# DDMAL/text_alignment

Measured on AMD Instinct MI355X. Metric: nw_dp_cells_per_s, higher is better.
Workload: dtype int32; 1 GPU; affine-gap NW, 4096 problems of 4096x4096 per GPU per step, default scoring [8,-4,-7,-7,-3,0], two-phase (score fill + windowed traceback); parallelism=problems sharded x1, no data-path collective, distinct_problems=256

## Files before the change

include/text_alignment_amd.h:

```cpp
#ifndef TEXT_ALIGNMENT_AMD_H
#define TEXT_ALIGNMENT_AMD_H

#include <stdint.h>

#ifdef __cplusplus
extern "C" {
#endif

#define TA_OK 0
#define TA_EINVAL (-1)
#define TA_ERANGE (-2)
#define TA_EHIP (-3)
#define TA_ELIMIT (-4)

#define TA_NW_FILL 1u
#define TA_NW_TRACEBACK 2u
#define TA_NW_CODES8 4u
#define TA_NW_WIDE 8u
#define TA_NW_NARROW 16u
#define TA_NW_OPENS_SAME 32u
#define TA_NW_ALPHABET_SHIFT 8
#define TA_NW_ALPHABET(a) (((uint32_t)(a) & 0xFFu) << TA_NW_ALPHABET_SHIFT)
#define TA_NW_ROWS_SHIFT 20
#define TA_NW_ROWS(r) (((uint32_t)(r) & 0x7u) << TA_NW_ROWS_SHIFT)
// ... 44 lines not shown
                      uint8_t* ws, const int64_t* ws_off,
                      uint8_t* ops_out, const int64_t* ops_off, int32_t* ops_len,
                      int32_t max_n, int32_t max_m, int64_t score_bound,
                      uint32_t flags, int32_t band_w, const int32_t* band_u, int32_t* band_ok, void* stream);
int ta_nw2_batch_funnel(const int32_t* t_codes, const int64_t* t_off,
                        const int32_t* o_codes, const int64_t* o_off, int32_t nprob,
                        const int32_t* params, int32_t params_stride,
                        uint8_t* ws, const int64_t* ws_off,
                        uint8_t* ops_out, const int64_t* ops_off, int32_t* ops_len,
                        int32_t max_n, int32_t max_m, int64_t score_bound,
                        uint32_t flags, int32_t band_w, const int32_t* band_u, int32_t* band_ok,
                        const int32_t* band_x0, int32_t* band_cert, void* stream);
int ta_nw2_funnel_plan(const int32_t* n_arr, const int32_t* m_arr, int32_t nprob, const int32_t* params,
                       int32_t params_stride, int32_t w, int32_t big, int32_t* x0_out, int32_t* ranges_out,
                       int32_t ranges_cap, int32_t* out);
int32_t ta_nw2_funnel_suf(int32_t rn, int32_t rm, const int32_t* params, int32_t* ap_out);
int32_t ta_nw2_band_bound(int32_t n, int32_t m, const int32_t* params, int32_t w);
int ta_nw2_band_plan(const int32_t* n_arr, const int32_t* m_arr, int32_t nprob, const int32_t* params,
                     int32_t params_stride, uint32_t flags, int32_t band, int32_t* out, int32_t* u_out,
                     int32_t* ranges_out, int32_t ranges_cap);

int32_t ta_nw2_traceback_plan(int32_t nprob, int32_t params_stride, uint32_t flags);
int ta_nw2_phase1_plan(int32_t max_n, int32_t max_m, uint32_t flags, int32_t* out);
int ta_nw2_phase1_plan_batch(int32_t max_n, int32_t max_m, int32_t nprob, uint32_t flags, int32_t* out);

int64_t ta_nw_general_score_bytes(int32_t n);
int64_t ta_nw_general_ptr_bytes(int32_t n, int32_t m);
int ta_nw_general(const int32_t* t, int32_t n, const int32_t* o, int32_t m,
                  const double* params, const double* table, int32_t tm,
                  double* score_ws, uint8_t* ptr_ws,
// ... 313 lines not shown
```

text_alignment_amd/csrc/nw_band.h:

```cpp
#pragma once
#include <stdint.h>

#include "nw_cell.h"

namespace ta {

constexpr int kBandSentinel = -(1 << 24);
constexpr int kBandMaxLen = 32768;
static_assert(((int64_t)kBandSentinel - 2ll * kBandMaxLen * 128 - (1 << 21)) * 64 > INT32_MIN, "sentinel-derived values, encoded");
struct BandRange { int gl, gh; };
TA_HD BandRange band_groups(int n, int m, int w, int s) {
    const int ngroups = PtrLayout<4>::ngroups(m);
    const int lo = (m < n ? m - n : 0) - w, hi = (m > n ? m - n : 0) + w;
    const int i0 = s * 256 + 1;
    const int jmin = i0 + lo > 1 ? i0 + lo : 1;
    const int jmax = i0 + 255 + hi < m ? i0 + 255 + hi : m;
    const int kmin = jmin - 1, kmax = jmax - 1 + 63;
    int gl = kmin >= 2 ? ((kmin - 2) / 64) * 16 - 16 : 0;
    if (gl < 0) gl = 0;
    int gh = (kmax / 64) * 16 + 32;
    if (gh >= ngroups || gh <= gl) gh = ngroups;
    if (gl >= gh) gl = 0;
    return BandRange{gl, gh};
}
// ... 22 lines not shown
    f.a = prm[0] > prm[1] ? prm[0] : prm[1];
    f.cvi = prm[4] + (prm[2] > 0 ? prm[2] : 0);
    f.chi = prm[5] + (prm[3] > 0 ? prm[3] : 0);
    f.ap = f.a > f.cvi ? f.a : f.cvi;
    if (f.chi > f.ap) f.ap = f.chi;
    return f;
}
template <typename T>
TA_HD T funnel_suf(T rn, T rm, const FunnelSys& f) {
    const T d = rn < rm ? rn : rm;
    const T none = rn * (T)f.cvi + rm * (T)f.chi;
    const T most = d * (T)f.a + (rn - d) * (T)f.cvi + (rm - d) * (T)f.chi;
    return none > most ? none : most;
}

TA_HD BandRange funnel_raw(int n, int m, const FunnelSys& f, int w_outer, int s) {
    const int64_t den_h = 2ll * ((int64_t)f.a - f.cvi - f.chi), den_l = (int64_t)f.a - 2ll * f.cvi - 2ll * f.chi;
    if (f.a <= 0 || den_h <= 0 || den_l <= 0) return BandRange{-1, -1};
    const int ngroups = PtrLayout<4>::ngroups(m);
    const int w0 = (n < m ? n : m) / 32 > 128 ? (n < m ? n : m) / 32 : 128;
    const int64_t num = (int64_t)f.a * (n - 256 * s);
    const int64_t wh = (num + den_h - 1) / den_h + w0, wl = (num + den_l - 1) / den_l + w0;
    const int off_lo = m < n ? m - n : 0, off_hi = m > n ? m - n : 0;
    const int lo = wl < w_outer ? off_lo - (int)wl : off_lo - w_outer;
    const int hi = wh < w_outer ? off_hi + (int)wh : off_hi + w_outer;
    const int i0 = s * 256 + 1;
    const int jmin = i0 + lo > 1 ? i0 + lo : 1;
    const int jmax = i0 + 255 + hi < m ? i0 + 255 + hi : m;
    const int kmin = jmin - 1, kmax = jmax - 1 + 63;
    int gl = kmin >= 2 ? ((kmin - 2) / 64) * 16 - 16 : 0;
    if (gl < 0) gl = 0;
    int gh = (kmax / 64) * 16 + 32;
    if (gh >= ngroups || gh <= gl) gh = ngroups;
    if (gl >= gh) gl = 0;
    return BandRange{gl, gh};
}
TA_HD bool funnel_ok(int n, int m, const FunnelSys& f, int w_outer) {
    const int nstrips = PtrLayout<4>::nstrips(n), ngroups = PtrLayout<4>::ngroups(m);
    BandRange prev{0, 0};
    for (int s = 0; s < nstrips; ++s) {
        const BandRange r = funnel_raw(n, m, f, w_outer, s);
        if (r.gl < 0) return false;
        if (s > 0) {
            if (r.gl < prev.gl || r.gh < prev.gh) return false;
            if (r.gl > 0 && prev.gh < ngroups && 4 * r.gl + 2 > 4 * prev.gh - 63) return false;
        }
        prev = r;
    }
    return true;
}
TA_HD BandRange funnel_groups(int n, int m, const int32_t* prm, int w_outer, int s) {
    const FunnelSys f = funnel_sys(prm);
    return funnel_ok(n, m, f, w_outer) ? funnel_raw(n, m, f, w_outer, s) : band_groups(n, m, w_outer, s);
}
inline bool funnel_ranges(int n, int m, const int32_t* prm, int w_outer, BandRange* rg) {
    const FunnelSys f = funnel_sys(prm);
    const bool own = funnel_ok(n, m, f, w_outer);
    const int nstrips = PtrLayout<4>::nstrips(n);
    for (int s = 0; s < nstrips; ++s) rg[s] = own ? funnel_raw(n, m, f, w_outer, s) : band_groups(n, m, w_outer, s);
    return own;
}

TA_HD int funnel_jlo(const BandRange& r, int i) { return r.gl == 0 ? 1 : 4 * r.gl - ((i - 1) % 256) / 4 + 3; }
TA_HD int funnel_jhi(const BandRange& r, int i, int m) {
    if (r.gh == PtrLayout<4>::ngroups(m)) return m;
    const int j = 4 * r.gh - ((i - 1) % 256) / 4;
    return j < m ? j : m;
}
inline int64_t funnel_exit0(int n, int m, const int32_t* prm, const BandRange* rg) {
    const FunnelSys f = funnel_sys(prm);
    int64_t best = -(1ll << 40);
    auto out = [&](int i, int j) {
        if (i < 1 || i > n || j < 1 || j > m) return false;
        const BandRange& r = rg[(i - 1) / 256];
        return j < funnel_jlo(r, i) || j > funnel_jhi(r, i, m);
    };
    auto take = [&](int64_t db, int i, int j) {
        if (out(i, j)) best = bmax(best, db + f.ap + funnel_suf<int64_t>(n - i, m - j, f));
    };
    for (int j = 0; j <= m; ++j) { take(-j, 1, j); take(-j, 1, j + 1); }
    for (int i = 1; i <= n; ++i) { take(-i, i, 1); take(-i, i + 1, 1); }
    return best;
}

}
```

text_alignment_amd/csrc/nw_hw.h:

```cpp
#pragma once
#include <hip/hip_runtime.h>
#include <stdint.h>

#include "nw_cell.h"

namespace ta {

struct NwArgs {
    const int32_t* t_codes; const int64_t* t_off;
    const int32_t* o_codes; const int64_t* o_off;
    const int32_t* params; int32_t params_stride;
    uint8_t* ws; const int64_t* ws_off;
    uint8_t* ops_out; const int64_t* ops_off; int32_t* ops_len;
    int32_t nprob;
    int32_t wide_stride;
    int32_t apad;
    int32_t band_w;
    const int32_t* band_u;
    int32_t* band_ok;
    int32_t* band_cert;
};
constexpr int kCertWords = 4;

__device__ __forceinline__ int v_max3(int a, int b, int c) {
    int d;
    asm("v_max3_i32 %0, %1, %2, %3" : "=v"(d) : "v"(a), "v"(b), "v"(c));
    return d;
}
__device__ __forceinline__ int v_and_or_x(int a, int mask) {
    int d;
    asm("v_and_or_b32 %0, %1, %2, 21" : "=v"(d) : "v"(a), "s"(mask));
    return d;
}
__device__ __forceinline__ unsigned v_bfi3(unsigned a, unsigned b) {
    unsigned d;
// ... 176 lines not shown
```

text_alignment_amd/csrc/ta_nw2.hip:

```cpp
#include <hip/hip_runtime.h>
#include <stdint.h>
#include <array>
#include <atomic>
#include <map>
#include <type_traits>
#include <vector>

#include "nw_band.h"
#include "nw_cell.h"
#include "nw_hw.h"
#include "ta_common.h"

namespace ta {

#ifndef TA_CK_GROUPS
#define TA_CK_GROUPS 16
#endif
constexpr int kCkGroups = TA_CK_GROUPS;
static_assert(kCkGroups % 4 == 0 && kCkGroups >= 4, "whole blocks of four groups");
constexpr int kStateInts = 10;
constexpr int kWsRange = 0x7ffff000;

#ifndef TA_SUBROWS
#define TA_SUBROWS 2
// ... 55 lines not shown
};

__device__ __forceinline__ int wave_max_i32(int v) {
#pragma unroll
    for (int o = 32; o > 0; o >>= 1) v = max(v, __shfl_xor(v, o));
    return __builtin_amdgcn_readfirstlane(v);
}
template <int W, int MODE, bool SAMEGO, typename OC, int BAND = 0>
__global__ __launch_bounds__(W * 64, MODE == 1 ? 5 : 2) void nw_score_kernel(NwArgs a) {
    constexpr int R = 4;
    using L = PtrLayout<R>;
    constexpr int SPG = L::SPG;
    constexpr bool PROFILE = (MODE == 2);
    using LC = typename std::conditional<PROFILE, uint16_t, OC>::type;
    constexpr int CHK = 4;
    constexpr bool FUNNEL = BAND == 3;
    extern __shared__ __attribute__((aligned(16))) unsigned char smem[];

    int p = blockIdx.x;
    if constexpr (BAND == 2) {
        if (a.band_ok[p] != 0) return;
    }
    const int64_t t0 = a.t_off[p], o0 = a.o_off[p];
    const int n = (int)(a.t_off[p + 1] - t0);
    const int m = (int)(a.o_off[p + 1] - o0);
    if (n <= 0 || m <= 0) return;

    const int32_t* prm = a.params + (size_t)p * a.params_stride;
    const CellConsts c = make_consts(prm[0], prm[1], prm[2], prm[3], prm[4], prm[5]);
    RawRegs kr;
    kr.cmis = prm[1] - prm[4] - prm[5]; kr.cmat = prm[0] - prm[4] - prm[5];
// ... 38 lines not shown

    const uint64_t wsa = reinterpret_cast<uint64_t>(ws_p);
    unsigned char* const ws_u = reinterpret_cast<unsigned char*>(
        ((uint64_t)(uint32_t)__builtin_amdgcn_readfirstlane((int)(wsa >> 32)) << 32) |
        (uint32_t)__builtin_amdgcn_readfirstlane((int)(uint32_t)wsa));
    const __amdgpu_buffer_rsrc_t wsrc = __builtin_amdgcn_make_buffer_rsrc(ws_u, 0, kWsRange, 0x00020000);
    const int nstrips = ws.nstrips, ngroups = ws.ngroups;
    const int prev_wave = (wave + W - 1) % W;
    const int g_lo = (63 + SPG - 1) / SPG;
    const int g_hi = (steady_ok && ws.total < kWsRange) ? ngroups : 0;
    const bool from_zero = PROFILE && g_hi > 0 && prm[4] <= -1;
    int pass = 0;
    const FunnelSys fsys = funnel_sys(prm);
    bool fun_ok = false;
    if constexpr (FUNNEL) fun_ok = a.band_cert[kCertWords * p + 3] != 0;
    auto strip_range = [&](int s_) { return fun_ok ? funnel_raw(n, m, fsys, a.band_w, s_) : band_groups(n, m, a.band_w, s_); };
    auto exit_of = [&](int db_hat, int i, int j, int i2, int j2) {
        return db_hat + prm[4] * i + prm[5] * j + fsys.ap + funnel_suf<int>(n - i2, m - j2, fsys);
    };
    int ex_wave = -(1 << 30), cnt_wave = 0;

    for (int s = wave; s < nstrips; s += W, ++pass) {
        int D[R], V[R], H[R], tc[R];
        const int row0 = s * L::SR + lane * R;
#pragma unroll
        for (int r = 0; r < R; ++r) {
            const int i = row0 + r + 1;
            D[r] = raw_of(bnd_D_col0(c, i));
            H[r] = raw_of(bnd_H_col0(c, i)) + yadj;
            V[r] = from_zero ? -(1 << 28) : 0;
            tc[r] = (i <= n) ? a.t_codes[t0 + i - 1] : -1;
        }
        int dsave = raw_of(bnd_D_col0(c, row0));
// ... 130 lines not shown
                    if (sub_last) hvo[j] = make_int2(V[R - 1], D[R - 1]);
                }
            }
            publish(g);
        };

        int g = 0;
        if ((BAND == 1 || FUNNEL) && gl > 0) {
            g = gl;
            wait_span(gl);
            if constexpr (FUNNEL) {
                const int gl_above = strip_range(s - 1).gl;
                const int c_lo = gl_above == 0 ? 1 : gl_above * SPG - 60;
                const int c_hi = min(m, gl * SPG + 2), i0 = s * L::SR + 1;
                int ex = -(1 << 30);
                for (int j = c_lo + lane; j <= c_hi; j += 64) {
                    const int db = hvd[j].y;
                    ex = max(ex, exit_of(db, i0 - 1, j, i0, j));
                    if (j + 1 <= c_hi) ex = max(ex, exit_of(db, i0 - 1, j, i0, j + 1));
                }
                ex_wave = max(ex_wave, wave_max_i32(ex));
                if (lane == 31) hvo[gl * SPG - 31] = make_int2(kBandSentinel, kBandSentinel);
            }
        } else {
            wait_span(0);
            load_group(0);
            const int e1 = from_zero ? 0 : min(g_lo, ngroups);
            for (; g < e1; ++g) group_edge(g);
        }

        int g_end = g_hi & ~3;
        if constexpr (BAND == 1 || FUNNEL) {
            g_end = min(g_end, g_fin);
            if (cert_strip) g_end = min(g_end, ((m - 1 + cert_lane) / SPG) & ~3);
// ... 99 lines not shown
#pragma unroll
                for (int b = 0; b < kCkGroups / CHK; ++b) block();
            }
            while (g < g_end) {
                checkpoint(g);
                block();
            }
            if (g < g_fin) {
                if ((g % CHK) == 0) wait_span(g);
                load_group(g);
            } else {
                if constexpr (FUNNEL) {
                    if (g_fin < ngroups) {
                        const int jr = g_fin * SPG - lane;
                        int ex = -(1 << 30);
                        if (jr <= m) {
#pragma unroll
                            for (int r = 0; r < R; ++r) {
                                const int i = row0 + 1 + r;
                                if (i > n) continue;
                                if (jr + 1 <= m) ex = max(ex, exit_of(D[r], i, jr, i, jr + 1));
                                if (jr + 1 <= m && i + 1 <= n) ex = max(ex, exit_of(D[r], i, jr, i + 1, jr + 1));
                                if (r == R - 1 && lane < 63 && i + 1 <= n) ex = max(ex, exit_of(D[r], i, jr, i + 1, jr));
                            }
                        }
                        if (jr + 1 <= m && row0 + 1 <= n) ex = max(ex, exit_of(dsave, row0, jr, row0 + 1, jr + 1));
                        ex_wave = max(ex_wave, wave_max_i32(ex));
                        int2* const row31 = reinterpret_cast<int2*>(ws_p + ws.row(s * kSubRows + 1)) + 1;
                        if (lane < 3 && g_fin * SPG - 30 + lane <= m)
                            row31[g_fin * SPG - 30 + lane] = make_int2(kBandSentinel, kBandSentinel);
                        int2* const rowp = reinterpret_cast<int2*>(ws_p + ws.row(s * kSubRows + kSubRows)) + 1;
                        const int c_hi = min(m, strip_range(s + 1).gh * SPG + 4);
                        for (int col = g_fin * SPG - 62 + lane; col <= c_hi; col += 64)
                            rowp[col] = make_int2(kBandSentinel, kBandSentinel);
                    }
                }
                if constexpr (BAND == 1) {
                    if (g_fin < ngroups) {
                        int2* const rowp = reinterpret_cast<int2*>(ws_p + ws.row(s * kSubRows + kSubRows)) + 1;
                        const int c_hi = min(m, band_groups(n, m, a.band_w, s + 1).gh * SPG + 4);
                        for (int col = g_fin * SPG - 62 + lane; col <= c_hi; col += 64)
// ... 26 lines not shown
    const bool own = n > 0 && m > 0 && n <= kBandMaxLen && m <= kBandMaxLen &&
                     funnel_ok(n, m, funnel_sys(a.params + (size_t)p * a.params_stride), a.band_w);
    a.band_cert[kCertWords * p] = INT32_MIN;
    a.band_cert[kCertWords * p + 1] = x0[p];
    a.band_cert[kCertWords * p + 2] = 0;
    a.band_cert[kCertWords * p + 3] = own ? 1 : 0;
    a.band_ok[p] = 0;
}
__global__ __launch_bounds__(256) void nw_band_certify_kernel(NwArgs a) {
    const int p = blockIdx.x * 256 + threadIdx.x;
    if (p >= a.nprob) return;
    const int n = (int)(a.t_off[p + 1] - a.t_off[p]);
    const int32_t* c = a.band_cert + kCertWords * (size_t)p;
    const bool ok = n > 0 && c[2] == PtrLayout<4>::nstrips(n) && c[0] > a.band_u[p] && c[0] > c[1];
    a.band_ok[p] = ok ? 1 : 0;
}

constexpr int kChunk = kCkGroups;
constexpr int kChunkGroups = kChunk + 1;
constexpr int kChunkSteps = kChunkGroups * 4;
#ifndef TA_TB2_LANES
#define TA_TB2_LANES 32
#endif
constexpr int kWinLanes = TA_TB2_LANES;
static_assert(kWinLanes >= 8 && kWinLanes <= 64, "window lanes");
constexpr int kHalfLanes = 32;
static_assert(kSubRows == 2 && kSubLanes == kHalfLanes, "nw_trace2h_kernel restarts half-strips: phase 1 must keep lane 31's rows");

#ifndef TA_P2_PROFILE
#define TA_P2_PROFILE 0
// ... 734 lines not shown
template <int W>
static hipError_t launch_score_funnel(const NwArgs& a, const int32_t* x0, size_t lds, bool samego, hipStream_t st) {
    const dim3 grid((a.nprob + 255) / 256);
    hipLaunchKernelGGL(nw_band_cert_init_kernel, grid, dim3(256), 0, st, a, x0);
    hipError_t e = hipGetLastError();
    if (e != hipSuccess) return e;
    e = samego ? launch_score_k<W, 2, true, uint16_t, 3>(a, lds, st) : launch_score_k<W, 2, false, uint16_t, 3>(a, lds, st);
    if (e != hipSuccess) return e;
    hipLaunchKernelGGL(nw_band_certify_kernel, grid, dim3(256), 0, st, a);
    e = hipGetLastError();
    if (e != hipSuccess) return e;
    return samego ? launch_score_k<W, 2, true, uint16_t, 2>(a, lds, st) : launch_score_k<W, 2, false, uint16_t, 2>(a, lds, st);
}

template <int W>
static hipError_t launch_score_w(const NwArgs& a, size_t lds, bool profile, bool samego, bool codes8, hipStream_t st) {
    if (profile) return samego ? launch_score_k<W, 2, true, uint16_t>(a, lds, st)
                               : launch_score_k<W, 2, false, uint16_t>(a, lds, st);
    return codes8 ? launch_score_k<W, 1, false, uint8_t>(a, lds, st)
                  : launch_score_k<W, 1, false, uint16_t>(a, lds, st);
}

constexpr size_t kLdsShared = 124 * 1024;
struct P1Plan { int mode, w, apad; size_t lds; bool samego, codes8; };

static P1Plan plan_phase1(int max_n, int max_m, uint32_t flags, int nprob = 1 << 20) {
    P1Plan pl{};
    const int nstrips = PtrLayout<4>::nstrips(max_n);
    const int wmax = nstrips >= 8 ? 8 : nstrips >= 4 ? 4 : nstrips >= 2 ? 2 : 1;
    pl.codes8 = (flags & TA_NW_CODES8) != 0;
// ... 181 lines not shown
                out[1] = (int32_t)(run * 1000 / ((int64_t)rg.size() * PtrLayout<4>::ngroups(m)));
            }
        }
    }
    return TA_OK;
}

static hipError_t launch_score(NwArgs a, int max_n, int max_m, uint32_t flags, hipStream_t st, const int32_t* band_x0 = nullptr) {
    const P1Plan pl = plan_phase1(max_n, max_m, flags, a.nprob);
    if (pl.lds > 160 * 1024) return hipErrorInvalidValue;
    a.apad = pl.apad;
    if (a.band_w > 0) {
        if (pl.mode != 2 || !a.band_u || !a.band_ok) return hipErrorInvalidValue;
        if (a.band_cert) {
            if (!band_x0) return hipErrorInvalidValue;
            if (pl.w == 8) return launch_score_funnel<8>(a, band_x0, pl.lds, pl.samego, st);
            if (pl.w == 4) return launch_score_funnel<4>(a, band_x0, pl.lds, pl.samego, st);
            return hipErrorInvalidValue;
        }
        if (pl.w == 8) return launch_score_band<8>(a, pl.lds, pl.samego, st);
        if (pl.w == 4) return launch_score_band<4>(a, pl.lds, pl.samego, st);
        return hipErrorInvalidValue;
    }
    switch (pl.w) {
    case 8: return launch_score_w<8>(a, pl.lds, pl.mode == 2, pl.samego, pl.codes8, st);
    case 4: return launch_score_w<4>(a, pl.lds, pl.mode == 2, pl.samego, pl.codes8, st);
    case 2: return launch_score_w<2>(a, pl.lds, pl.mode == 2, pl.samego, pl.codes8, st);
    default: return launch_score_w<1>(a, pl.lds, pl.mode == 2, pl.samego, pl.codes8, st);
    }
}
// ... 56 lines not shown
                                 uint8_t* ops_out, const int64_t* ops_off, int32_t* ops_len,
                                 int32_t max_n, int32_t max_m, int64_t score_bound,
                                 uint32_t flags, int32_t band_w, const int32_t* band_u, int32_t* band_ok, void* stream) {
    return ta_nw2_batch_funnel(t_codes, t_off, o_codes, o_off, nprob, params, params_stride, ws, ws_off, ops_out, ops_off,
                               ops_len, max_n, max_m, score_bound, flags, band_w, band_u, band_ok, nullptr, nullptr, stream);
}

extern "C" int ta_nw2_batch_funnel(const int32_t* t_codes, const int64_t* t_off,
                                   const int32_t* o_codes, const int64_t* o_off, int32_t nprob,
                                   const int32_t* params, int32_t params_stride,
                                   uint8_t* ws, const int64_t* ws_off,
                                   uint8_t* ops_out, const int64_t* ops_off, int32_t* ops_len,
                                   int32_t max_n, int32_t max_m, int64_t score_bound,
                                   uint32_t flags, int32_t band_w, const int32_t* band_u, int32_t* band_ok,
                                   const int32_t* band_x0, int32_t* band_cert, void* stream) {
    if ((band_x0 == nullptr) != (band_cert == nullptr) || (band_cert && band_w < 2))
        return ta_fail(TA_EINVAL, "funnel: the exit words' host part and the certificate array, with a band width >= 2, or neither");
    if (nprob < 0 || max_n < 0 || max_m < 0) return ta_fail(TA_EINVAL, "negative size");
    if (band_w < 0 || (band_w > 0 && (!band_u || !band_ok || band_w == 1)))
        return ta_fail(TA_EINVAL, "band: width >= 2 with its bound and list arrays, or 0");
    if (nprob == 0) return TA_OK;
    if (!t_off || !o_off || !params || !ws_off || !ops_off || !ops_len)
        return ta_fail(TA_EINVAL, "null pointer argument");
    if (params_stride != 0 && params_stride != 6) return ta_fail(TA_EINVAL, "params_stride must be 0 or 6");
    if (score_bound < 0 || score_bound >= (1ll << 23))
        return ta_fail(TA_ERANGE, "(n+m+2)*max|param| does not fit the 32-bit encoded scores");
    if (max_m > ta_nw2_max_m()) return ta_fail(TA_ELIMIT, "m exceeds the LDS capacity for the OCR codes");
    hipStream_t st = reinterpret_cast<hipStream_t>(stream);
    NwArgs a{t_codes, t_off, o_codes, o_off, params, params_stride, ws, ws_off,
             ops_out, ops_off, ops_len, nprob};
    a.band_w = band_w; a.band_u = band_u; a.band_ok = band_ok; a.band_cert = band_cert;
    if ((flags & TA_NW_FILL) && max_n > 0 && max_m > 0) {
        if (!t_codes || !o_codes || !ws) return ta_fail(TA_EINVAL, "null code/workspace pointer");
        if (flags & TA_NW_CHECK_IDS) {
            const int rc = check_ids(a, flags, st);
            if (rc != TA_OK) return rc;
        }
        const hipError_t e = launch_score(a, max_n, max_m, flags, st, band_x0);
        if (e != hipSuccess) return ta_fail_hip(e, "nw_score_kernel launch");
    }
    if (flags & TA_NW_TRACEBACK) {
        if (!ops_out && (max_n + max_m) > 0) return ta_fail(TA_EINVAL, "null ops_out");
        {
            const hipError_t em = hipMemsetAsync(ops_len, 0xFF, sizeof(int32_t) * (size_t)nprob, st);
            if (em != hipSuccess) return ta_fail_hip(em, "ops_len reset");
        }
// ... 13 lines not shown
```

text_alignment_amd/textSeqCompare.py:

```python
import numpy as np
import torch

from . import _native

default_match = 10
default_mismatch = -5
gap_open = -10
gap_extend = -1
default_sys = [8, -4, -7, -7, -3, 0]

GAP = '_'


def parse_scoring_system(scoring_system):
    if scoring_system is None:
        scoring_system = default_sys
    size = len(scoring_system)
    if size == 5 and callable(scoring_system[0]):
        return [0, 0] + [scoring_system[k] for k in range(1, 5)], scoring_system[0]
    if size == 6:
        return [scoring_system[k] for k in range(6)], None
    if size == 4:
        hit, miss, opn, ext = (scoring_system[k] for k in range(4))
        return [hit, miss, opn, opn, ext, ext], None
# ... 144 lines not shown
            flags |= self.phase1_flags()
        if self.wide is not None and not self.two_phase:
            flags |= _native.TA_NW_WIDE if self.wide else _native.TA_NW_NARROW
        if self.rows and not self.two_phase:
            flags |= (int(self.rows) & 0x7) << _native.TA_NW_ROWS_SHIFT
        stream = torch.cuda.current_stream(self.device).cuda_stream
        args = (self.t_codes.data_ptr(), self.t_off.data_ptr(),
                self.o_codes.data_ptr(), self.o_off.data_ptr(), self.nprob,
                self.params.data_ptr(), self.params_stride,
                self.ws.data_ptr(), self.ws_off.data_ptr(),
                self.ops.data_ptr(), self.ops_off.data_ptr(), self.ops_len.data_ptr(),
                self.max_n, self.max_m, self.score_bound, flags)
        if self.two_phase:
            plan = self.band_plan(flags)
            if plan["w"] > 0 and plan["shape"] == "funnel":
                rc = _native.lib.ta_nw2_batch_funnel(*args, plan["w"], plan["u_dev"].data_ptr(), plan["ok_dev"].data_ptr(),
                                                     plan["x0_dev"].data_ptr(), plan["cert_dev"].data_ptr(), stream)
            elif plan["w"] > 0:
                rc = _native.lib.ta_nw2_batch_band(*args, plan["w"], plan["u_dev"].data_ptr(), plan["ok_dev"].data_ptr(), stream)
            else:
                rc = _native.lib.ta_nw2_batch(*args, stream)
        else:
            rc = _native.lib.ta_nw_batch(*args, stream)
        _native.check(rc, "ta_nw2_batch" if self.two_phase else "ta_nw_batch")

    def band_plan(self, flags=None):
        if self.band_shape not in ("auto", "uniform", "funnel"):
            raise ValueError("band_shape must be 'auto', 'uniform' or 'funnel'")
        if flags is None:
            flags = (_native.TA_NW_CODES8 if self.codes8 else 0) | self.phase1_flags()
        key = (int(self.band), int(flags) & ~(_native.TA_NW_FILL | _native.TA_NW_TRACEBACK), self.band_shape)
        if self._band_plan is not None and self._band_plan["key"] == key:
            return self._band_plan
        n32, m32 = self.n.astype(np.int32), self.m.astype(np.int32)
        out = np.zeros(8, dtype=np.int32)
        u = np.zeros(max(self.nprob, 1), dtype=np.int32)
        ranges = np.zeros(2 * ((self.max_n + 255) // 256 + 1), dtype=np.int32)
        rc = _native.lib.ta_nw2_band_plan(n32.ctypes.data, m32.ctypes.data, self.nprob, self._params_host.ctypes.data,
                                          self.params_stride, key[1], key[0], out.ctypes.data, u.ctypes.data,
                                          ranges.ctypes.data, len(ranges))
        _native.check(rc, "ta_nw2_band_plan")
        plan = {"key": key, "w": int(out[0]), "rule_w": int(out[1]), "share": out[2] / 1000.0, "largest": int(out[4]),
                "ranges": [(int(ranges[2 * k]), int(ranges[2 * k + 1])) for k in range(int(out[3]))], "u": u,
                "shape": "uniform"}
        funnel = plan["w"] > 0 and (self.band_shape == "funnel" or (self.band_shape == "auto" and out[5] == 1))
        if plan["w"] > 0:
            uni = np.zeros(len(ranges), dtype=np.int32)
            out_u = np.zeros(8, dtype=np.int32)
            rc = _native.lib.ta_nw2_band_plan(n32.ctypes.data, m32.ctypes.data, self.nprob, self._params_host.ctypes.data,
                                              self.params_stride, key[1], plan["w"], out_u.ctypes.data, None,
                                              uni.ctypes.data, len(uni))
            _native.check(rc, "ta_nw2_band_plan")
            plan["uniform_share"] = out_u[2] / 1000.0
            if not funnel:
                plan["share"] = plan["uniform_share"]
                plan["ranges"] = [(int(uni[2 * k]), int(uni[2 * k + 1])) for k in range(int(out[3]))]
        if funnel:
            x0 = np.zeros(max(self.nprob, 1), dtype=np.int32)
            fout = np.zeros(4, dtype=np.int32)
            rc = _native.lib.ta_nw2_funnel_plan(n32.ctypes.data, m32.ctypes.data, self.nprob, self._params_host.ctypes.data,
                                                self.params_stride, plan["w"], plan["largest"], x0.ctypes.data,
                                                ranges.ctypes.data, len(ranges), fout.ctypes.data)
            _native.check(rc, "ta_nw2_funnel_plan")
            plan.update(shape="funnel", x0=x0, share=fout[1] / 1000.0, funnel_own_ranges=bool(fout[0]),
                        ranges=[(int(ranges[2 * k]), int(ranges[2 * k + 1])) for k in range(int(out[3]))])
        if plan["w"] > 0:
            (plan["u_dev"],) = _native.upload_packed([u], self.device)
            plan["ok_dev"] = torch.zeros(self.nprob, dtype=torch.int32, device=self.device)
            if funnel:
                (plan["x0_dev"],) = _native.upload_packed([plan["x0"]], self.device)
                plan["cert_dev"] = torch.zeros(4 * self.nprob, dtype=torch.int32, device=self.device)
        self._band_plan = plan
        return plan

    def band_fallbacks(self):
        plan = self._band_plan
        if not self.two_phase or plan is None or plan["w"] <= 0:
            return []
        return [int(k) for k in np.nonzero(plan["ok_dev"].cpu().numpy() == 0)[0]]

    def band_certificate(self):
        plan = self._band_plan
        if not self.two_phase or plan is None or plan["w"] <= 0 or plan["shape"] != "funnel":
            return None
        return plan["cert_dev"].cpu().numpy().reshape(self.nprob, 4)[:, :3]

# ... 220 lines not shown
```

Baseline: 7863 billion cells/s.

## Tighten funnel band using per-problem bit-parallel LCS suffix bounds

Adds a funnel-lcs band mode. A bit-parallel LCS pre-pass computes suffix LCS lengths per problem, and those lengths give a tighter upper bound on the remaining score. The funnel can then be shrunk to a 25% scale and exit checks stay valid, so the fill phase computes fewer cells. The cost is an extra per-problem kernel, a workspace table, and extra work in the exit-bound evaluation. It becomes the default path when band_shape is auto/funnel-lcs, the alphabet is at most 64 and m is at most 4096.

Measured after the change: 8310 billion cells/s, median of 6. 5.7% higher.

```diff
diff --git a/include/text_alignment_amd.h b/include/text_alignment_amd.h
--- a/include/text_alignment_amd.h
+++ b/include/text_alignment_amd.h
@@ -82,6 +82,20 @@
 int ta_nw2_funnel_plan(const int32_t* n_arr, const int32_t* m_arr, int32_t nprob, const int32_t* params,
                        int32_t params_stride, int32_t w, int32_t big, int32_t* x0_out, int32_t* ranges_out,
                        int32_t ranges_cap, int32_t* out);
+int ta_nw2_batch_funnel_lcs(const int32_t* t_codes, const int64_t* t_off,
+                            const int32_t* o_codes, const int64_t* o_off, int32_t nprob,
+                            const int32_t* params, int32_t params_stride,
+                            uint8_t* ws, const int64_t* ws_off,
+                            uint8_t* ops_out, const int64_t* ops_off, int32_t* ops_len,
+                            int32_t max_n, int32_t max_m, int64_t score_bound,
+                            uint32_t flags, int32_t band_w, const int32_t* band_u, int32_t* band_ok,
+                            const int32_t* band_x0, int32_t* band_cert, int32_t* lcs, void* stream);
+int64_t ta_nw2_funnel_lcs_words(int32_t nprob, int32_t max_n);
+int32_t ta_nw2_funnel_lcs_scale_pm(void);
+int32_t ta_nw2_funnel_lcs_max_m(void);
+int ta_nw2_funnel_ranges(int32_t n, int32_t m, const int32_t* params, int32_t w, int32_t scale_pm,
+                         int32_t* ranges_out, int32_t ranges_cap, int32_t* out);
+int32_t ta_nw2_funnel_suf_lcs(int32_t rn, int32_t rm, int32_t l, const int32_t* params);
 int32_t ta_nw2_funnel_suf(int32_t rn, int32_t rm, const int32_t* params, int32_t* ap_out);
 int32_t ta_nw2_band_bound(int32_t n, int32_t m, const int32_t* params, int32_t w);
 int ta_nw2_band_plan(const int32_t* n_arr, const int32_t* m_arr, int32_t nprob, const int32_t* params,
diff --git a/text_alignment_amd/csrc/nw_band.h b/text_alignment_amd/csrc/nw_band.h
--- a/text_alignment_amd/csrc/nw_band.h
+++ b/text_alignment_amd/csrc/nw_band.h
@@ -60,12 +60,19 @@
     return none > most ? none : most;
 }
 
+constexpr int kFunnelFullPm = 1000;
+#ifndef TA_FUNNEL_LCS_SCALE_PM
+#define TA_FUNNEL_LCS_SCALE_PM 250
+#endif
+constexpr int kFunnelLcsScalePm = TA_FUNNEL_LCS_SCALE_PM;
+template <int PM = kFunnelFullPm>
 TA_HD BandRange funnel_raw(int n, int m, const FunnelSys& f, int w_outer, int s) {
     const int64_t den_h = 2ll * ((int64_t)f.a - f.cvi - f.chi), den_l = (int64_t)f.a - 2ll * f.cvi - 2ll * f.chi;
     if (f.a <= 0 || den_h <= 0 || den_l <= 0) return BandRange{-1, -1};
     const int ngroups = PtrLayout<4>::ngroups(m);
     const int w0 = (n < m ? n : m) / 32 > 128 ? (n < m ? n : m) / 32 : 128;
-    const int64_t num = (int64_t)f.a * (n - 256 * s);
+    const int64_t full = (int64_t)f.a * (n - 256 * s);
+    const int64_t num = PM == kFunnelFullPm ? full : (full * PM + 999) / 1000;
     const int64_t wh = (num + den_h - 1) / den_h + w0, wl = (num + den_l - 1) / den_l + w0;
     const int off_lo = m < n ? m - n : 0, off_hi = m > n ? m - n : 0;
     const int lo = wl < w_outer ? off_lo - (int)wl : off_lo - w_outer;
@@ -81,11 +88,12 @@
     if (gl >= gh) gl = 0;
     return BandRange{gl, gh};
 }
+template <int PM = kFunnelFullPm>
 TA_HD bool funnel_ok(int n, int m, const FunnelSys& f, int w_outer) {
     const int nstrips = PtrLayout<4>::nstrips(n), ngroups = PtrLayout<4>::ngroups(m);
     BandRange prev{0, 0};
     for (int s = 0; s < nstrips; ++s) {
-        const BandRange r = funnel_raw(n, m, f, w_outer, s);
+        const BandRange r = funnel_raw<PM>(n, m, f, w_outer, s);
         if (r.gl < 0) return false;
         if (s > 0) {
             if (r.gl < prev.gl || r.gh < prev.gh) return false;
@@ -99,11 +107,12 @@
     const FunnelSys f = funnel_sys(prm);
     return funnel_ok(n, m, f, w_outer) ? funnel_raw(n, m, f, w_outer, s) : band_groups(n, m, w_outer, s);
 }
+template <int PM = kFunnelFullPm>
 inline bool funnel_ranges(int n, int m, const int32_t* prm, int w_outer, BandRange* rg) {
     const FunnelSys f = funnel_sys(prm);
-    const bool own = funnel_ok(n, m, f, w_outer);
+    const bool own = funnel_ok<PM>(n, m, f, w_outer);
     const int nstrips = PtrLayout<4>::nstrips(n);
-    for (int s = 0; s < nstrips; ++s) rg[s] = own ? funnel_raw(n, m, f, w_outer, s) : band_groups(n, m, w_outer, s);
+    for (int s = 0; s < nstrips; ++s) rg[s] = own ? funnel_raw<PM>(n, m, f, w_outer, s) : band_groups(n, m, w_outer, s);
     return own;
 }
 
@@ -129,4 +138,34 @@
     return best;
 }
 
+struct FunnelLcs { int mat, mis; };
+TA_HD FunnelLcs funnel_lcs_sys(const int32_t* prm) { return FunnelLcs{prm[0], prm[1]}; }
+template <typename T>
+TA_HD T funnel_suf_lcs(T rn, T rm, T l, const FunnelSys& f, const FunnelLcs& q) {
+    const T stat = funnel_suf<T>(rn, rm, f);
+    if (q.mis >= q.mat) return stat;
+    const T d = rn < rm ? rn : rm;
+    const T lp = l < d ? (l < 0 ? 0 : l) : d;
+    const T none = rn * (T)f.cvi + rm * (T)f.chi;
+    const T all_match = lp * (T)q.mat + (rn - lp) * (T)f.cvi + (rm - lp) * (T)f.chi;
+    const T most = lp * (T)q.mat + (d - lp) * (T)q.mis + (rn - d) * (T)f.cvi + (rm - d) * (T)f.chi;
+    T best = none > all_match ? none : all_match;
+    if (most > best) best = most;
+    return best < stat ? best : stat;
 }
+
+constexpr int kLcsMaxM = 4096;
+constexpr int kLcsMaxAlphabet = 64;
+
+TA_HD int lcs_row_off(int max_n) { return (max_n + 1 + 63) & ~63; }
+TA_HD int64_t lcs_stride(int max_n) { return (int64_t)lcs_row_off(max_n) + 192ll * PtrLayout<4>::nstrips(max_n); }
+TA_HD int lcs_row_at(const int32_t* row, int m, int j) {
+    const int c = m - j;
+    if (c <= 0) return 0;
+    const int w = c >> 6, b = c & 63;
+    if (w >= 64) return row[128 + 63] + __builtin_popcountll(((const uint64_t*)row)[63]);
+    const uint64_t bits = ((const uint64_t*)row)[w];
+    return row[128 + w] + (b ? __builtin_popcountll(bits & ((1ull << b) - 1)) : 0);
+}
+
+}
diff --git a/text_alignment_amd/csrc/nw_hw.h b/text_alignment_amd/csrc/nw_hw.h
--- a/text_alignment_amd/csrc/nw_hw.h
+++ b/text_alignment_amd/csrc/nw_hw.h
@@ -19,6 +19,8 @@
     const int32_t* band_u;
     int32_t* band_ok;
     int32_t* band_cert;
+    int32_t* lcs;
+    int32_t lcs_max_n;
 };
 constexpr int kCertWords = 4;
 
diff --git a/text_alignment_amd/csrc/ta_nw2.hip b/text_alignment_amd/csrc/ta_nw2.hip
--- a/text_alignment_amd/csrc/ta_nw2.hip
+++ b/text_alignment_amd/csrc/ta_nw2.hip
@@ -93,7 +93,8 @@
     constexpr bool PROFILE = (MODE == 2);
     using LC = typename std::conditional<PROFILE, uint16_t, OC>::type;
     constexpr int CHK = 4;
-    constexpr bool FUNNEL = BAND == 3;
+    constexpr bool FUNNEL = BAND == 3 || BAND == 4;
+    constexpr bool LCS = BAND == 4;
     extern __shared__ __attribute__((aligned(16))) unsigned char smem[];
 
     int p = blockIdx.x;
@@ -162,9 +163,22 @@
     const FunnelSys fsys = funnel_sys(prm);
     bool fun_ok = false;
     if constexpr (FUNNEL) fun_ok = a.band_cert[kCertWords * p + 3] != 0;
-    auto strip_range = [&](int s_) { return fun_ok ? funnel_raw(n, m, fsys, a.band_w, s_) : band_groups(n, m, a.band_w, s_); };
+    bool lcs_on = false;
+    if constexpr (LCS) lcs_on = a.band_cert[kCertWords * p + 3] == 2;
+    auto strip_range = [&](int s_) {
+        if constexpr (LCS)
+            if (lcs_on) return funnel_raw<kFunnelLcsScalePm>(n, m, fsys, a.band_w, s_);
+        return fun_ok ? funnel_raw(n, m, fsys, a.band_w, s_) : band_groups(n, m, a.band_w, s_);
+    };
     auto exit_of = [&](int db_hat, int i, int j, int i2, int j2) {
         return db_hat + prm[4] * i + prm[5] * j + fsys.ap + funnel_suf<int>(n - i2, m - j2, fsys);
+    };
+    const FunnelLcs lsys = funnel_lcs_sys(prm);
+    const int32_t* const lcs_p = LCS && lcs_on ? a.lcs + (size_t)p * lcs_stride(a.lcs_max_n) : nullptr;
+    auto exit_at = [&](int db_hat, int i, int j, int i2, int j2, int l) {
+        if constexpr (LCS)
+            return db_hat + prm[4] * i + prm[5] * j + fsys.ap + funnel_suf_lcs<int>(n - i2, m - j2, l, fsys, lsys);
+        else return exit_of(db_hat, i, j, i2, j2);
     };
     int ex_wave = -(1 << 30), cnt_wave = 0;
 
@@ -325,10 +339,12 @@
                 const int c_lo = gl_above == 0 ? 1 : gl_above * SPG - 60;
                 const int c_hi = min(m, gl * SPG + 2), i0 = s * L::SR + 1;
                 int ex = -(1 << 30);
+                const int32_t* const lrow = lcs_p ? lcs_p + lcs_row_off(a.lcs_max_n) + 192 * s : nullptr;
                 for (int j = c_lo + lane; j <= c_hi; j += 64) {
                     const int db = hvd[j].y;
-                    ex = max(ex, exit_of(db, i0 - 1, j, i0, j));
-                    if (j + 1 <= c_hi) ex = max(ex, exit_of(db, i0 - 1, j, i0, j + 1));
+                    const int l = lrow ? lcs_row_at(lrow, m, j) : kBandMaxLen;
+                    ex = max(ex, exit_at(db, i0 - 1, j, i0, j, l));
+                    if (j + 1 <= c_hi) ex = max(ex, exit_at(db, i0 - 1, j, i0, j + 1, l));
                 }
                 ex_wave = max(ex_wave, wave_max_i32(ex));
                 if (lane == 31) hvo[gl * SPG - 31] = make_int2(kBandSentinel, kBandSentinel);
@@ -458,17 +474,23 @@
                     if (g_fin < ngroups) {
                         const int jr = g_fin * SPG - lane;
                         int ex = -(1 << 30);
+                        const int l = lcs_p && jr <= m && row0 < n ? lcs_p[64 * s + lane] : kBandMaxLen;
+                        bool diag_in = false;
+                        if constexpr (LCS) {
+                            const BandRange nx = strip_range(s + 1);
+                            diag_in = lane == 63 && jr + 1 >= (nx.gl == 0 ? 1 : nx.gl * SPG + 3) && jr + 1 <= min(m, nx.gh * SPG);
+                        }
                         if (jr <= m) {
 #pragma unroll
                             for (int r = 0; r < R; ++r) {
                                 const int i = row0 + 1 + r;
                                 if (i > n) continue;
-                                if (jr + 1 <= m) ex = max(ex, exit_of(D[r], i, jr, i, jr + 1));
-                                if (jr + 1 <= m && i + 1 <= n) ex = max(ex, exit_of(D[r], i, jr, i + 1, jr + 1));
-                                if (r == R - 1 && lane < 63 && i + 1 <= n) ex = max(ex, exit_of(D[r], i, jr, i + 1, jr));
+                                if (jr + 1 <= m) ex = max(ex, exit_at(D[r], i, jr, i, jr + 1, l));
+                                if (jr + 1 <= m && i + 1 <= n && !(r == R - 1 && diag_in)) ex = max(ex, exit_at(D[r], i, jr, i + 1, jr + 1, l));
+                                if (r == R - 1 && lane < 63 && i + 1 <= n) ex = max(ex, exit_at(D[r], i, jr, i + 1, jr, l));
                             }
                         }
-                        if (jr + 1 <= m && row0 + 1 <= n) ex = max(ex, exit_of(dsave, row0, jr, row0 + 1, jr + 1));
+                        if (jr + 1 <= m && row0 + 1 <= n) ex = max(ex, exit_at(dsave, row0, jr, row0 + 1, jr + 1, l));
                         ex_wave = max(ex_wave, wave_max_i32(ex));
                         int2* const row31 = reinterpret_cast<int2*>(ws_p + ws.row(s * kSubRows + 1)) + 1;
                         if (lane < 3 && g_fin * SPG - 30 + lane <= m)
@@ -525,6 +547,173 @@
     const int32_t* c = a.band_cert + kCertWords * (size_t)p;
     const bool ok = n > 0 && c[2] == PtrLayout<4>::nstrips(n) && c[0] > a.band_u[p] && c[0] > c[1];
     a.band_ok[p] = ok ? 1 : 0;
+}
+
+__global__ __launch_bounds__(256) void nw_band_cert_init_lcs_kernel(NwArgs a, const int32_t* x0, int alphabet) {
+    const int p = blockIdx.x * 256 + threadIdx.x;
+    if (p >= a.nprob) return;
+    const int n = (int)(a.t_off[p + 1] - a.t_off[p]), m = (int)(a.o_off[p + 1] - a.o_off[p]);
+    const int32_t* prm = a.params + (size_t)p * a.params_stride;
+    const FunnelSys f = funnel_sys(prm);
+    const bool sized = n > 0 && m > 0 && n <= kBandMaxLen && m <= kBandMaxLen;
+    const bool lcs = sized && n >= 2 && m <= kLcsMaxM && n <= a.lcs_max_n && alphabet > 0 && alphabet <= kLcsMaxAlphabet &&
+                     prm[0] > prm[1] && funnel_ok<kFunnelLcsScalePm>(n, m, f, a.band_w);
+    const bool own = lcs || (sized && funnel_ok(n, m, f, a.band_w));
+    a.band_cert[kCertWords * p] = INT32_MIN;
+    a.band_cert[kCertWords * p + 1] = lcs ? -(1 << 30) : x0[p];
+    a.band_cert[kCertWords * p + 2] = lcs ? -1 : 0;
+    a.band_cert[kCertWords * p + 3] = lcs ? 2 : own ? 1 : 0;
+    a.band_ok[p] = 0;
+}
+
+__global__ __launch_bounds__(64) void nw_lcs_suffix_kernel(NwArgs a, int alphabet) {
+    extern __shared__ __attribute__((aligned(16))) unsigned char smem[];
+    const int p = blockIdx.x;
+    if (a.band_cert[kCertWords * p + 3] != 2) return;
+    const int64_t t0 = a.t_off[p], o0 = a.o_off[p];
+    const int n = (int)(a.t_off[p + 1] - t0), m = (int)(a.o_off[p + 1] - o0);
+    const int32_t* prm = a.params + (size_t)p * a.params_stride;
+    const FunnelSys fsys = funnel_sys(prm);
+    const FunnelLcs lsys = funnel_lcs_sys(prm);
+    const int lane = threadIdx.x;
+    const int nstrips = PtrLayout<4>::nstrips(n), ngroups = PtrLayout<4>::ngroups(m);
+    uint64_t* const mask = reinterpret_cast<uint64_t*>(smem);
+    int* const rg = reinterpret_cast<int*>(smem + (size_t)(alphabet + 1) * 512);
+    int32_t* const out = a.lcs + (size_t)p * lcs_stride(a.lcs_max_n);
+    int32_t* const rows = out + lcs_row_off(a.lcs_max_n);
+
+    for (int k = 0; k <= alphabet; ++k) mask[k * 64 + lane] = 0;
+    for (int b0 = 0; b0 < 64; b0 += 16) {
+        int syms[16];
+#pragma unroll
+        for (int k = 0; k < 16; ++k) {
+            const int c = 64 * lane + b0 + k;
+            syms[k] = c < m ? a.o_codes[o0 + m - 1 - c] : -1;
+        }
+#pragma unroll
+        for (int k = 0; k < 16; ++k)
+            if ((unsigned)syms[k] < (unsigned)alphabet) mask[syms[k] * 64 + lane] |= 1ull << (b0 + k);
+    }
+    for (int s = lane; s < nstrips; s += 64) {
+        const BandRange r = funnel_raw<kFunnelLcsScalePm>(n, m, fsys, a.band_w, s);
+        rg[2 * s] = r.gl; rg[2 * s + 1] = r.gh;
+    }
+    for (int k = lane; k < 64 * nstrips; k += 64) out[k] = 0;
+    __threadfence();
+    __syncthreads();
+    auto is_out = [&](int i, int j) {
+        if (i < 1 || i > n || j < 1 || j > m) return false;
+        const BandRange r{rg[2 * ((i - 1) / 256)], rg[2 * ((i - 1) / 256) + 1]};
+        return j < funnel_jlo(r, i) || j > funnel_jhi(r, i, m);
+    };
+    auto exit0 = [&](int db, int i2, int j2, int l) {
+        return db + fsys.ap + funnel_suf_lcs<int>(n - i2, m - j2, l, fsys, lsys);
+    };
+
+    int ev_s = nstrips, ev_l = -1, ev_t = -1, ev_w = 0, ev_b = 0, ev_gh = 0;
+    auto next_event = [&]() {
+        while (true) {
+            if (--ev_l < 0) {
+                ev_l = 63;
+                if (--ev_s < 0) { ev_t = -1; return; }
+                ev_gh = __builtin_amdgcn_readfirstlane(rg[2 * ev_s + 1]);
+            }
+            if (ev_gh >= ngroups) { ev_l = 0; continue; }
+            const int r = n - 256 * ev_s - 4 * ev_l, cnt = m - 4 * ev_gh + ev_l;
+            if (r < 1 || cnt < 0) continue;
+            ev_w = cnt >> 6; ev_b = cnt & 63; ev_t = r - 1 + ev_w;
+            return;
+        }
+    };
+    next_event();
+
+    const int pad = alphabet * 512;
+    const unsigned char* const mask_lane = smem + lane * 8;
+    auto load_feed = [&](int base) {
+        const int tk = n - 1 - base - lane;
+        int f = pad;
+        if (tk >= 0) { const int c = a.t_codes[t0 + tk]; f = (unsigned)c < (unsigned)alphabet ? c * 512 : pad; }
+        return f;
+    };
+    uint64_t V = ~0ull;
+    int cy = 0, nc = 0, ex = -(1 << 30);
+    int feed = load_feed(0);
+    int symn = __builtin_amdgcn_update_dpp(feed, pad, 0x138, 0xf, 0xf, false);
+    uint64_t Mn = *reinterpret_cast<const uint64_t*>(mask_lane + symn);
+    const int nchunks = (n + 63 + 63) / 64;
+    auto step = [&](int t, auto rows_tag, int row_ta, int row_tb, int i_row) {
+        constexpr bool ROWS = decltype(rows_tag)::value;
+        const int sym = symn;
+        const uint64_t M = Mn;
+        symn = __builtin_amdgcn_update_dpp(feed, sym, 0x138, 0xf, 0xf, false);
+        Mn = *reinterpret_cast<const uint64_t*>(mask_lane + symn);
+        const int cin = __builtin_amdgcn_update_dpp(0, cy, 0x138, 0xf, 0xf, true);
+        const int nin = __builtin_amdgcn_update_dpp(0, nc, 0x138, 0xf, 0xf, true);
+        const uint64_t U = V & M;
+        const uint64_t sum = V + U + (uint64_t)(unsigned)cin;
+        const uint32_t sh = (uint32_t)(sum >> 32), uh = (uint32_t)(U >> 32), vh = (uint32_t)(V >> 32);
+        cy = (int)(((sh & uh) | (~sh & vh)) >> 31);
+        V = sum | (V & ~M);
+        nc = nin + __builtin_popcountll(V);
+        if (t == ev_t) {
+            if (lane == ev_w) out[64 * ev_s + ev_l] = 64 * ev_w - nin + __builtin_popcountll(~V & ((1ull << ev_b) - 1));
+            next_event();
+        }
+        if constexpr (ROWS) {
+            const unsigned da = (unsigned)(t - row_ta), db = (unsigned)(t - row_tb);
+            if (da < 64u || db < 64u) {
+                if (lane == (int)(da < 64u ? da : db)) {
+                    int32_t* const row = rows + 192 * ((da < 64u ? i_row : i_row + 256) >> 8);
+                    reinterpret_cast<uint64_t*>(row)[lane] = ~V;
+                    row[128 + lane] = 64 * lane - nin;
+                }
+            }
+        }
+    };
+    for (int ch = 0; ch < nchunks; ++ch) {
+        const int base = ch * 64;
+        const int feed_next = load_feed(base + 64);
+        const int i_row = ((n - base - 1) >> 8) << 8;
+        const int row_ta = i_row >= 0 ? n - i_row - 1 : -(1 << 30);
+        const int row_tb = i_row + 256 < n ? n - i_row - 257 : -(1 << 30);
+        const bool rows_here = (unsigned)(base + 63 - row_ta) < 127u || (unsigned)(base + 63 - row_tb) < 127u;
+        auto chunk = [&](auto rows_tag) {
+#pragma unroll 1
+            for (int q = 0; q < 63; q += 3) {
+#pragma unroll
+                for (int k = 0; k < 3; ++k) {
+                    feed = __builtin_amdgcn_update_dpp(feed, feed, 0x134, 0xf, 0xf, false);
+                    step(base + q + k, rows_tag, row_ta, row_tb, i_row);
+                }
+            }
+            feed = feed_next;
+            step(base + 63, rows_tag, row_ta, row_tb, i_row);
+        };
+        if (rows_here) chunk(std::true_type{}); else chunk(std::false_type{});
+        const int ltot = 64 * 64 - __builtin_amdgcn_readlane(nc, 63);
+        const int r = base + 1 - lane, i = n - r;
+        if (r >= 0 && r <= n) {
+            if (is_out(i, 1)) ex = max(ex, exit0(-i, i, 1, ltot));
+            if (is_out(i + 1, 1)) ex = max(ex, exit0(-i, i + 1, 1, ltot));
+        }
+    }
+    const int pc = 64 * (lane + 1) - nc;
+    {
+        const int before = pc - __builtin_popcountll(~V);
+        for (int b = 0; b < 64; ++b) {
+            const int cnt = 64 * lane + b, j = m - cnt;
+            if (j < 0) break;
+            const int l = before + (b ? __builtin_popcountll(~V & ((1ull << b) - 1)) : 0);
+            if (is_out(1, j)) ex = max(ex, exit0(-j, 1, j, l));
+            if (is_out(1, j + 1)) ex = max(ex, exit0(-j, 1, j + 1, l));
+        }
+    }
+    ex = wave_max_i32(ex);
+    if (lane == 0) {
+        atomicMax(&a.band_cert[kCertWords * p + 1], ex);
+        __threadfence();
+        atomicAdd(&a.band_cert[kCertWords * p + 2], 1);
+    }
 }
 
 constexpr int kChunk = kCkGroups;
@@ -1289,6 +1478,28 @@
 }
 
 template <int W>
+static hipError_t launch_score_funnel_lcs(const NwArgs& a, const int32_t* x0, size_t lds, bool samego, int alphabet,
+                                          hipStream_t st) {
+    const dim3 grid((a.nprob + 255) / 256);
+    const bool covers = alphabet > 0 && alphabet <= kLcsMaxAlphabet;
+    hipLaunchKernelGGL(nw_band_cert_init_lcs_kernel, grid, dim3(256), 0, st, a, x0, covers ? alphabet : 0);
+    hipError_t e = hipGetLastError();
+    if (e != hipSuccess) return e;
+    if (covers) {
+        const size_t lcs_lds = (size_t)(alphabet + 1) * 512 + 8 * (size_t)PtrLayout<4>::nstrips(a.lcs_max_n);
+        hipLaunchKernelGGL(nw_lcs_suffix_kernel, dim3(a.nprob), dim3(64), lcs_lds, st, a, alphabet);
+        e = hipGetLastError();
+        if (e != hipSuccess) return e;
+    }
+    e = samego ? launch_score_k<W, 2, true, uint16_t, 4>(a, lds, st) : launch_score_k<W, 2, false, uint16_t, 4>(a, lds, st);
+    if (e != hipSuccess) return e;
+    hipLaunchKernelGGL(nw_band_certify_kernel, grid, dim3(256), 0, st, a);
+    e = hipGetLastError();
+    if (e != hipSuccess) return e;
+    return samego ? launch_score_k<W, 2, true, uint16_t, 2>(a, lds, st) : launch_score_k<W, 2, false, uint16_t, 2>(a, lds, st);
+}
+
+template <int W>
 static hipError_t launch_score_w(const NwArgs& a, size_t lds, bool profile, bool samego, bool codes8, hipStream_t st) {
     if (profile) return samego ? launch_score_k<W, 2, true, uint16_t>(a, lds, st)
                                : launch_score_k<W, 2, false, uint16_t>(a, lds, st);
@@ -1500,6 +1711,12 @@
         if (pl.mode != 2 || !a.band_u || !a.band_ok) return hipErrorInvalidValue;
         if (a.band_cert) {
             if (!band_x0) return hipErrorInvalidValue;
+            if (a.lcs) {
+                const int alphabet = (int)((flags >> TA_NW_ALPHABET_SHIFT) & 0xFFu);
+                if (pl.w == 8) return launch_score_funnel_lcs<8>(a, band_x0, pl.lds, pl.samego, alphabet, st);
+                if (pl.w == 4) return launch_score_funnel_lcs<4>(a, band_x0, pl.lds, pl.samego, alphabet, st);
+                return hipErrorInvalidValue;
+            }
             if (pl.w == 8) return launch_score_funnel<8>(a, band_x0, pl.lds, pl.samego, st);
             if (pl.w == 4) return launch_score_funnel<4>(a, band_x0, pl.lds, pl.samego, st);
             return hipErrorInvalidValue;
@@ -1586,6 +1803,50 @@
                                    int32_t max_n, int32_t max_m, int64_t score_bound,
                                    uint32_t flags, int32_t band_w, const int32_t* band_u, int32_t* band_ok,
                                    const int32_t* band_x0, int32_t* band_cert, void* stream) {
+    return ta_nw2_batch_funnel_lcs(t_codes, t_off, o_codes, o_off, nprob, params, params_stride, ws, ws_off, ops_out, ops_off,
+                                   ops_len, max_n, max_m, score_bound, flags, band_w, band_u, band_ok, band_x0, band_cert,
+                                   nullptr, stream);
+}
+
+extern "C" int64_t ta_nw2_funnel_lcs_words(int32_t nprob, int32_t max_n) {
+    if (nprob < 0 || max_n < 0 || max_n > kBandMaxLen) return -1;
+    return (int64_t)nprob * lcs_stride(max_n);
+}
+extern "C" int ta_nw2_funnel_ranges(int32_t n, int32_t m, const int32_t* params, int32_t w, int32_t scale_pm,
+                                    int32_t* ranges_out, int32_t ranges_cap, int32_t* out) {
+    if (!params || n <= 0 || m <= 0 || n > kBandMaxLen || m > kBandMaxLen || w < 2 ||
+        (scale_pm != kFunnelFullPm && scale_pm != kFunnelLcsScalePm))
+        return ta_fail(TA_EINVAL, "bad argument (scale_pm: 1000 or ta_nw2_funnel_lcs_scale_pm())");
+    std::vector<BandRange> rg(PtrLayout<4>::nstrips(n));
+    const bool own = scale_pm == kFunnelFullPm ? funnel_ranges(n, m, params, w, rg.data())
+                                               : funnel_ranges<kFunnelLcsScalePm>(n, m, params, w, rg.data());
+    int64_t run = 0;
+    for (size_t s = 0; s < rg.size(); ++s) {
+        run += rg[s].gh - rg[s].gl;
+        if (ranges_out && 2 * (int)s + 1 < ranges_cap) { ranges_out[2 * s] = rg[s].gl; ranges_out[2 * s + 1] = rg[s].gh; }
+    }
+    if (out) {
+        out[0] = own ? 1 : 0;
+        out[1] = (int32_t)(run * 1000 / ((int64_t)rg.size() * PtrLayout<4>::ngroups(m)));
+    }
+    return TA_OK;
+}
+extern "C" int32_t ta_nw2_funnel_lcs_scale_pm(void) { return kFunnelLcsScalePm; }
+extern "C" int32_t ta_nw2_funnel_lcs_max_m(void) { return kLcsMaxM; }
+extern "C" int32_t ta_nw2_funnel_suf_lcs(int32_t rn, int32_t rm, int32_t l, const int32_t* params) {
+    if (!params || rn < 0 || rm < 0 || l < 0) return INT32_MAX;
+    return clamp_i32(funnel_suf_lcs<int64_t>(rn, rm, l, funnel_sys(params), funnel_lcs_sys(params)));
+}
+
+extern "C" int ta_nw2_batch_funnel_lcs(const int32_t* t_codes, const int64_t* t_off,
+                                       const int32_t* o_codes, const int64_t* o_off, int32_t nprob,
+                                       const int32_t* params, int32_t params_stride,
+                                       uint8_t* ws, const int64_t* ws_off,
+                                       uint8_t* ops_out, const int64_t* ops_off, int32_t* ops_len,
+                                       int32_t max_n, int32_t max_m, int64_t score_bound,
+                                       uint32_t flags, int32_t band_w, const int32_t* band_u, int32_t* band_ok,
+                                       const int32_t* band_x0, int32_t* band_cert, int32_t* lcs, void* stream) {
+    if (lcs && !band_cert) return ta_fail(TA_EINVAL, "funnel-lcs: the table goes with the funnel's certificate array");
     if ((band_x0 == nullptr) != (band_cert == nullptr) || (band_cert && band_w < 2))
         return ta_fail(TA_EINVAL, "funnel: the exit words' host part and the certificate array, with a band width >= 2, or neither");
     if (nprob < 0 || max_n < 0 || max_m < 0) return ta_fail(TA_EINVAL, "negative size");
@@ -1602,6 +1863,7 @@
     NwArgs a{t_codes, t_off, o_codes, o_off, params, params_stride, ws, ws_off,
              ops_out, ops_off, ops_len, nprob};
     a.band_w = band_w; a.band_u = band_u; a.band_ok = band_ok; a.band_cert = band_cert;
+    a.lcs = max_n <= kBandMaxLen ? lcs : nullptr; a.lcs_max_n = max_n;
     if ((flags & TA_NW_FILL) && max_n > 0 && max_m > 0) {
         if (!t_codes || !o_codes || !ws) return ta_fail(TA_EINVAL, "null code/workspace pointer");
         if (flags & TA_NW_CHECK_IDS) {
diff --git a/text_alignment_amd/textSeqCompare.py b/text_alignment_amd/textSeqCompare.py
--- a/text_alignment_amd/textSeqCompare.py
+++ b/text_alignment_amd/textSeqCompare.py
@@ -182,8 +182,9 @@
         if self.two_phase:
             plan = self.band_plan(flags)
             if plan["w"] > 0 and plan["shape"] == "funnel":
-                rc = _native.lib.ta_nw2_batch_funnel(*args, plan["w"], plan["u_dev"].data_ptr(), plan["ok_dev"].data_ptr(),
-                                                     plan["x0_dev"].data_ptr(), plan["cert_dev"].data_ptr(), stream)
+                rc = _native.lib.ta_nw2_batch_funnel_lcs(*args, plan["w"], plan["u_dev"].data_ptr(), plan["ok_dev"].data_ptr(),
+                                                         plan["x0_dev"].data_ptr(), plan["cert_dev"].data_ptr(),
+                                                         plan["lcs_dev"].data_ptr() if plan["lcs"] else None, stream)
             elif plan["w"] > 0:
                 rc = _native.lib.ta_nw2_batch_band(*args, plan["w"], plan["u_dev"].data_ptr(), plan["ok_dev"].data_ptr(), stream)
             else:
@@ -193,8 +194,8 @@
         _native.check(rc, "ta_nw2_batch" if self.two_phase else "ta_nw_batch")
 
     def band_plan(self, flags=None):
-        if self.band_shape not in ("auto", "uniform", "funnel"):
-            raise ValueError("band_shape must be 'auto', 'uniform' or 'funnel'")
+        if self.band_shape not in ("auto", "uniform", "funnel", "funnel-lcs"):
+            raise ValueError("band_shape must be 'auto', 'uniform', 'funnel' or 'funnel-lcs'")
         if flags is None:
             flags = (_native.TA_NW_CODES8 if self.codes8 else 0) | self.phase1_flags()
         key = (int(self.band), int(flags) & ~(_native.TA_NW_FILL | _native.TA_NW_TRACEBACK), self.band_shape)
@@ -211,7 +212,7 @@
         plan = {"key": key, "w": int(out[0]), "rule_w": int(out[1]), "share": out[2] / 1000.0, "largest": int(out[4]),
                 "ranges": [(int(ranges[2 * k]), int(ranges[2 * k + 1])) for k in range(int(out[3]))], "u": u,
                 "shape": "uniform"}
-        funnel = plan["w"] > 0 and (self.band_shape == "funnel" or (self.band_shape == "auto" and out[5] == 1))
+        funnel = plan["w"] > 0 and (self.band_shape in ("funnel", "funnel-lcs") or (self.band_shape == "auto" and out[5] == 1))
         if plan["w"] > 0:
             uni = np.zeros(len(ranges), dtype=np.int32)
             out_u = np.zeros(8, dtype=np.int32)
@@ -231,13 +232,30 @@
                                                 ranges.ctypes.data, len(ranges), fout.ctypes.data)
             _native.check(rc, "ta_nw2_funnel_plan")
             plan.update(shape="funnel", x0=x0, share=fout[1] / 1000.0, funnel_own_ranges=bool(fout[0]),
-                        ranges=[(int(ranges[2 * k]), int(ranges[2 * k + 1])) for k in range(int(out[3]))])
+                        ranges=[(int(ranges[2 * k]), int(ranges[2 * k + 1])) for k in range(int(out[3]))], lcs=False)
+            alphabet = (int(flags) >> _native.TA_NW_ALPHABET_SHIFT) & 0xFF
+            if self.band_shape != "funnel" and 0 < alphabet <= 64:
+                plan["lcs"] = True
+                plan["static_share"] = plan["share"]
+                big = plan["largest"]
+                prm_big = np.ascontiguousarray(self._params_host[big if self.params_stride else 0])
+                if m32[big] <= _native.lib.ta_nw2_funnel_lcs_max_m() and prm_big[0] > prm_big[1]:
+                    rc = _native.lib.ta_nw2_funnel_ranges(int(n32[big]), int(m32[big]), prm_big.ctypes.data, plan["w"],
+                                                          _native.lib.ta_nw2_funnel_lcs_scale_pm(), ranges.ctypes.data,
+                                                          len(ranges), fout.ctypes.data)
+                    _native.check(rc, "ta_nw2_funnel_ranges")
+                    if fout[0]:
+                        plan.update(share=fout[1] / 1000.0,
+                                    ranges=[(int(ranges[2 * k]), int(ranges[2 * k + 1])) for k in range(int(out[3]))])
         if plan["w"] > 0:
             (plan["u_dev"],) = _native.upload_packed([u], self.device)
             plan["ok_dev"] = torch.zeros(self.nprob, dtype=torch.int32, device=self.device)
             if funnel:
                 (plan["x0_dev"],) = _native.upload_packed([plan["x0"]], self.device)
                 plan["cert_dev"] = torch.zeros(4 * self.nprob, dtype=torch.int32, device=self.device)
+                if plan["lcs"]:
+                    words = int(_native.lib.ta_nw2_funnel_lcs_words(self.nprob, self.max_n))
+                    plan["lcs_dev"] = torch.empty(max(words, 16), dtype=torch.int32, device=self.device)
         self._band_plan = plan
         return plan
 
```
